# emilemathieu/RiemannHamiltonianMonteCarlo

Hardware: AMD Instinct MI355X
Metric: leapfrog-steps/sec (whole node) (higher is better)
Workload: dtype f64 (the two O(M D^2) contractions as exact int8-sliced integer GEMMs)

## Files before the change

### riemannhamiltonianmontecarlo_amd/csrc/kernels.hip.h

```cpp
#pragma once
#include <hip/hip_runtime.h>
#include <stdint.h>
#include "plan.h"

typedef double d4 __attribute__((ext_vector_type(4)));

#define RM_PI2 6.283185307179586476925286766559
#define RM_PK_DOUBLES (2688 + 64)
template <bool PK>
__device__ __forceinline__ int rm_row(int i) {
  if (!PK) return i * RM_LD;
  const int I = i >> 4;
  return (128 * I + 160) * I + (i & 15) * (16 * I + 18);
}
template <bool PK>
__device__ __forceinline__ int rm_len(int i) { return PK ? 16 * ((i >> 4) + 1) : 64; }

struct DevData {
  const double* Xr;
  const double* Xt;
  const double* t;
  int M, Mp, D, DP, nblk;
  double inv_alpha;
  double log_prior_const;
// ... 584 lines not shown
  }
  double* __restrict__ G = Gq + (size_t)blockIdx.y * plane_stride + (size_t)c * DP * DP;
  int t = 0;
#pragma unroll
  for (int I = 0; I < NB; ++I)
#pragma unroll
    for (int J = I; J < NB; ++J) {
#pragma unroll
      for (int r = 0; r < 4; ++r) {
        const int row = NB * (rr + 4 * r) + I;
        const int col = NB * ci + J;
        double val = acc[t][r];
        if (row == col && blockIdx.y == 0) val += dd.inv_alpha;
        if (I != J || row >= col) {
          G[row * DP + col] = val;
          G[col * DP + row] = val;
        }
      }
      ++t;
    }
}

typedef float f4 __attribute__((ext_vector_type(4)));
template <int NB>
__global__ __launch_bounds__(256) void k_assemble_f32(DevData dd, int n_chains, const int* __restrict__ phase,
                                                      const double* __restrict__ vrow, double* __restrict__ Gq, int nbk) {
  const int DP = dd.DP;
  const int lane = threadIdx.x & 63;
  const int c = blockIdx.x * 4 + (threadIdx.x >> 6);
  if (c >= n_chains) return;
  if (phase[c] != 1) return;
  int bA = 0, bB = 0;
  if (nbk > 1) {
    while ((bB + 1) * (bB + 2) / 2 <= (int)blockIdx.y) ++bB;
    bA = blockIdx.y - bB * (bB + 1) / 2;
  }
  const bool diag = (bA == bB);
  const int WB = 16 * NB;
  const int rr = lane >> 4, ci = lane & 15;
  const double* __restrict__ xpA = dd.Xr + (size_t)rr * DP + WB * bA + NB * ci;
  const double* __restrict__ xpB = dd.Xr + (size_t)rr * DP + WB * bB + NB * ci;
  const double* __restrict__ vp = vrow + (size_t)c * dd.Mp + rr;
  f4 acc[NB][NB];
#pragma unroll
  for (int I = 0; I < NB; ++I)
#pragma unroll
    for (int J = 0; J < NB; ++J) acc[I][J] = (f4){0.f, 0.f, 0.f, 0.f};
  for (int n1 = 0; n1 < dd.Mp; n1 += 16)
#pragma unroll
  for (int n0 = n1; n0 < n1 + 16; n0 += 4) {
    float xa[NB], xb[NB];
    const float vv = (float)vp[n0];
#pragma unroll
    for (int I = 0; I < NB; ++I) {
      xa[I] = vv * (float)xpA[(size_t)n0 * DP + I];
      xb[I] = (float)xpB[(size_t)n0 * DP + I];
    }
#pragma unroll
    for (int I = 0; I < NB; ++I)
#pragma unroll
      for (int J = 0; J < NB; ++J)
        if (!diag || J >= I) acc[I][J] = __builtin_amdgcn_mfma_f32_16x16x4f32(xa[I], xb[J], acc[I][J], 0, 0, 0);
  }
  double* __restrict__ G = Gq + (size_t)c * DP * DP;
#pragma unroll
  for (int I = 0; I < NB; ++I)
#pragma unroll
    for (int J = 0; J < NB; ++J) {
      if (diag && J < I) continue;
#pragma unroll
      for (int r = 0; r < 4; ++r) {
        const int row = WB * bA + NB * (4 * rr + r) + I;
        const int col = WB * bB + NB * ci + J;
        double val = (double)acc[I][J][r];
        if (row == col) val += dd.inv_alpha;
        if (!diag || I != J || row >= col) {
          G[(size_t)row * DP + col] = val;
          G[(size_t)col * DP + row] = val;
        }
      }
    }
}

template <int NB, int CM, bool TRV = false>
__device__ __forceinline__ void mompass_body(const DevData& dd, int n_chains, int nsplit, const double* __restrict__ wq,
                                             const double* __restrict__ uq, double* __restrict__ qpart, d4* __restrict__ ctile,
                                             const double* __restrict__ R = nullptr, double* __restrict__ trpart = nullptr) {
  static_assert(!TRV || CM == 2, "the trace product rides on the pass that loads its c tiles");
  constexpr int DP = 16 * NB;
  constexpr int KK = DP / 4;
  const int lane = threadIdx.x & 63;
  const int c0 = (blockIdx.x * 4 + __builtin_amdgcn_readfirstlane((int)(threadIdx.x >> 6))) * 16;
  if (c0 >= n_chains) return;
  const int split = blockIdx.y;
  const int rr = lane >> 4, ci = lane & 15;
  const int cj = min(c0 + ci, n_chains - 1);
  double Wb[CM == 2 ? 1 : KK], Ub[KK];
#pragma unroll
  for (int kk = 0; kk < KK; ++kk) {
    if (CM != 2) Wb[kk] = wq[(size_t)cj * DP + 4 * kk + rr];
    Ub[kk] = uq[(size_t)cj * DP + 4 * kk + rr];
  }
  __shared__ double s_u[TRV ? 4 * KK * 64 : 1];
  double* const my_u = s_u + (TRV ? ((threadIdx.x >> 6) * KK) * 64 + lane : 0);
  if constexpr (TRV) {
#pragma unroll
    for (int kk = 0; kk < KK; ++kk) my_u[kk * 64] = Ub[kk];
  }
  const brsrc rXt = buf_rsrc(dd.Xt), rXr = buf_rsrc(dd.Xr), rR = buf_rsrc(TRV ? R + (size_t)c0 * dd.Mp : nullptr);
  const unsigned r_off = (unsigned)((cj - c0) * dd.Mp + 8 * rr) * 8u;
  d4 T[TRV ? NB : 1];
  if constexpr (TRV) {
#pragma unroll
    for (int I = 0; I < NB; ++I) T[I] = (d4){0.0, 0.0, 0.0, 0.0};
  }
  const int nb16 = dd.Mp / 16, nb32 = dd.Mp / 32;
  const int per = (nb32 + nsplit - 1) / nsplit;
  const int B0 = split * per, B1 = min(nb32, B0 + per);
  d4* __restrict__ ct = ctile + (size_t)(c0 >> 4) * nb16 * 64 + lane;
  const brsrc rC = buf_rsrc(ctile + (size_t)(c0 >> 4) * nb16 * 64);
  const unsigned c_off = (unsigned)lane * 32u;
  auto load_c = [&](int t) { return buf_d4(rC, c_off, (unsigned)t * 2048u); };
  d4 Q[NB];
#pragma unroll
  for (int I = 0; I < NB; ++I) Q[I] = (d4){0.0, 0.0, 0.0, 0.0};
  const unsigned xt_off = (unsigned)(rr * dd.Mp + 2 * rm_perm16(ci)) * 8u;
  const unsigned xr_off = (unsigned)(8 * rr * DP + NB * ci) * 8u;
  d2 A[KK];
  d4 ccA = (d4){0.0, 0.0, 0.0, 0.0}, ccB = ccA;
  auto load_a = [&](int B, int k0, int k1) {
#pragma unroll
    for (int kk = 0; kk < KK; ++kk)
      if (kk >= k0 && kk < k1) A[kk] = buf_d2(rXt, xt_off, (unsigned)(4 * kk * dd.Mp + B * 32) * 8u);
  };
  auto xrow4 = [&](int n, double (&x)[NB]) { buf_dn<NB>(rXr, xr_off, (unsigned)(n * DP) * 8u, x); };
  if constexpr (CM == 2) {
    double xa[4][NB], xb[4][NB];
    d4 h0 = (d4){0.0, 0.0, 0.0, 0.0}, h1 = h0;
    if (B0 < B1) {
      load_a(B0, 0, KK);
      ccA = load_c(2 * B0);
      ccB = load_c(2 * B0 + 1);
#pragma unroll
      for (int r = 0; r < 4; ++r) xrow4(32 * B0 + 2 * r, xa[r]);
#pragma unroll
      for (int r = 0; r < 4; ++r) xrow4(32 * B0 + 2 * r + 1, xb[r]);
    }
    for (int B = B0; B < B1; ++B) {
      const int Bn = B + 1 < B1 ? B + 1 : B, n1 = 32 * Bn;
      d4 SA = (d4){0.0, 0.0, 0.0, 0.0}, SB = SA;
      if constexpr (TRV) { h0 = buf_d4(rR, r_off, (unsigned)(32 * B) * 8u); h1 = buf_d4(rR, r_off + 32u, (unsigned)(32 * B) * 8u); }
#pragma unroll
      for (int kk = 0; kk < KK; ++kk) {
        const double uk = TRV ? my_u[kk * 64] : Ub[kk];
        SA = __builtin_amdgcn_mfma_f64_16x16x4f64(A[kk].x, uk, SA, 0, 0, 0);
        SB = __builtin_amdgcn_mfma_f64_16x16x4f64(A[kk].y, uk, SB, 0, 0, 0);
        A[kk] = buf_d2(rXt, xt_off, (unsigned)(4 * kk * dd.Mp + Bn * 32) * 8u);
        __builtin_amdgcn_sched_barrier(0);
      }
      double RA[4], RB[4], TA[TRV ? 4 : 1], TB[TRV ? 4 : 1];
#pragma unroll
      for (int r = 0; r < 4; ++r) {
        RA[r] = ccA[r] * SA[r] * SA[r];
        RB[r] = ccB[r] * SB[r] * SB[r];
        if constexpr (TRV) {
          TA[r] = ccA[r] * (r < 2 ? h0[2 * r] : h1[2 * r - 4]);
          TB[r] = ccB[r] * (r < 2 ? h0[2 * r + 1] : h1[2 * r - 3]);
        }
      }
      __builtin_amdgcn_sched_barrier(0);
      ccA = load_c(2 * Bn);
      ccB = load_c(2 * Bn + 1);
      __builtin_amdgcn_sched_barrier(0);
#pragma unroll
      for (int r = 0; r < 4; ++r) {
#pragma unroll
        for (int I = 0; I < NB; ++I) Q[I] = __builtin_amdgcn_mfma_f64_16x16x4f64(xa[r][I], RA[r], Q[I], 0, 0, 0);
        if constexpr (TRV) {
#pragma unroll
          for (int I = 0; I < NB; ++I) T[I] = __builtin_amdgcn_mfma_f64_16x16x4f64(xa[r][I], TA[r], T[I], 0, 0, 0);
        }
        xrow4(n1 + 2 * r, xa[r]);
        __builtin_amdgcn_sched_barrier(0);
      }
#pragma unroll
      for (int r = 0; r < 4; ++r) {
#pragma unroll
        for (int I = 0; I < NB; ++I) Q[I] = __builtin_amdgcn_mfma_f64_16x16x4f64(xb[r][I], RB[r], Q[I], 0, 0, 0);
        if constexpr (TRV) {
#pragma unroll
          for (int I = 0; I < NB; ++I) T[I] = __builtin_amdgcn_mfma_f64_16x16x4f64(xb[r][I], TB[r], T[I], 0, 0, 0);
        }
        xrow4(n1 + 2 * r + 1, xb[r]);
        __builtin_amdgcn_sched_barrier(0);
      }
    }
  } else {
  if (B0 < B1) {
    load_a(B0, 0, KK);
  }
  for (int B = B0; B < B1; ++B) {
    const int n0 = 32 * B;
    double xa[4][NB], xb[4][NB];
    if (CM == 2) {
#pragma unroll
      for (int r = 0; r < 4; ++r) xrow4(n0 + 2 * r, xa[r]);
      __builtin_amdgcn_sched_barrier(0);
    }
    d4 FA = (d4){0.0, 0.0, 0.0, 0.0}, FB = FA, SA = FA, SB = FA;
#pragma unroll
    for (int kk = 0; kk < KK; ++kk) {
      if (CM != 2) {
        FA = __builtin_amdgcn_mfma_f64_16x16x4f64(A[kk].x, Wb[kk], FA, 0, 0, 0);
        FB = __builtin_amdgcn_mfma_f64_16x16x4f64(A[kk].y, Wb[kk], FB, 0, 0, 0);
      }
      const double uk = TRV ? my_u[kk * 64] : Ub[kk];
      SA = __builtin_amdgcn_mfma_f64_16x16x4f64(A[kk].x, uk, SA, 0, 0, 0);
      SB = __builtin_amdgcn_mfma_f64_16x16x4f64(A[kk].y, uk, SB, 0, 0, 0);
    }
    d4 cA = ccA, cB = ccB;
    d4 h0 = (d4){0.0, 0.0, 0.0, 0.0}, h1 = h0;
    if constexpr (TRV) { h0 = buf_d4(rR, r_off, (unsigned)n0 * 8u); h1 = buf_d4(rR, r_off + 32u, (unsigned)n0 * 8u); }
    __builtin_amdgcn_sched_barrier(0);
#pragma unroll
    for (int r = 0; r < 4; ++r) {
      if (CM == 2) xrow4(n0 + 2 * r + 1, xb[r]);
      else xrow4(n0 + 2 * r, xa[r]);
    }
    if (B + 1 < B1) load_a(B + 1, 0, KK / 2);
    __builtin_amdgcn_sched_barrier(0);
    if (CM != 2) {
      d4 pa, va;
      sigmoid4(FA, pa, va, cA);
      if (CM == 1) ct[(size_t)(2 * B) * 64] = cA;
    }
#pragma unroll
    for (int r = 0; r < 4; ++r) {
      const double RA = cA[r] * SA[r] * SA[r];
#pragma unroll
      for (int I = 0; I < NB; ++I) Q[I] = __builtin_amdgcn_mfma_f64_16x16x4f64(xa[r][I], RA, Q[I], 0, 0, 0);
      if constexpr (TRV) {
        const double TA = cA[r] * (r < 2 ? h0[2 * r] : h1[2 * r - 4]);
#pragma unroll
        for (int I = 0; I < NB; ++I) T[I] = __builtin_amdgcn_mfma_f64_16x16x4f64(xa[r][I], TA, T[I], 0, 0, 0);
      }
    }
    __builtin_amdgcn_sched_barrier(0);
    if (CM != 2) {
#pragma unroll
      for (int r = 0; r < 4; ++r) xrow4(n0 + 2 * r + 1, xb[r]);
    }
    if (B + 1 < B1) {
      load_a(B + 1, KK / 2, KK);
      if (CM == 2) { ccA = load_c(2 * B + 2); ccB = load_c(2 * B + 3); }
    }
    __builtin_amdgcn_sched_barrier(0);
    if (CM != 2) {
      d4 pb, vb;
      sigmoid4(FB, pb, vb, cB);
      if (CM == 1) ct[(size_t)(2 * B + 1) * 64] = cB;
    }
#pragma unroll
    for (int r = 0; r < 4; ++r) {
      const double RB = cB[r] * SB[r] * SB[r];
#pragma unroll
      for (int I = 0; I < NB; ++I) Q[I] = __builtin_amdgcn_mfma_f64_16x16x4f64(xb[r][I], RB, Q[I], 0, 0, 0);
      if constexpr (TRV) {
        const double TB = cB[r] * (r < 2 ? h0[2 * r + 1] : h1[2 * r - 3]);
#pragma unroll
        for (int I = 0; I < NB; ++I) T[I] = __builtin_amdgcn_mfma_f64_16x16x4f64(xb[r][I], TB, T[I], 0, 0, 0);
      }
    }
  }
  }
  if (c0 + ci < n_chains) {
    double* __restrict__ out = qpart + ((size_t)split * n_chains + c0 + ci) * DP;
#pragma unroll
    for (int I = 0; I < NB; ++I)
#pragma unroll
      for (int r = 0; r < 4; ++r) {
        const int d = NB * (rr + 4 * r) + I;
        if (d < dd.D) out[d] = Q[I][r];
      }
    if constexpr (TRV) {
      double* __restrict__ tout = trpart + ((size_t)split * n_chains + c0 + ci) * DP;
#pragma unroll
      for (int I = 0; I < NB; ++I)
#pragma unroll
        for (int r = 0; r < 4; ++r) {
          const int d = NB * (rr + 4 * r) + I;
          if (d < dd.D) tout[d] = T[I][r];
        }
    }
  }
}
template <int NB>
__global__ __launch_bounds__(256, 2) void k_mompass_trv(DevData dd, int n_chains, int nsplit, const double* __restrict__ uq, double* __restrict__ qpart,
                                                     d4* __restrict__ ctile, const double* __restrict__ R, double* __restrict__ trpart) {
  mompass_body<NB, 2, true>(dd, n_chains, nsplit, nullptr, uq, qpart, ctile, R, trpart);
}
template <int NB, int CM>
__global__ __launch_bounds__(256, 2) void k_mompass(DevData dd, int n_chains, int nsplit, const double* __restrict__ wq,
                                                 const double* __restrict__ uq, double* __restrict__ qpart, d4* __restrict__ ctile,
                                                 const int* __restrict__ cstale = nullptr) {
  if constexpr (CM == 3) {
    const int c0 = (blockIdx.x * 4 + (threadIdx.x >> 6)) * 16;
    if (c0 >= n_chains) return;
    const int c = c0 + (threadIdx.x & 15);
    const bool stale = __builtin_amdgcn_ballot_w64(c < n_chains && cstale[min(c, n_chains - 1)] != 0) != 0ull;
    if (stale) mompass_body<NB, 1>(dd, n_chains, nsplit, wq, uq, qpart, ctile);
    else mompass_body<NB, 2>(dd, n_chains, nsplit, wq, uq, qpart, ctile);
  } else {
    mompass_body<NB, CM>(dd, n_chains, nsplit, wq, uq, qpart, ctile);
  }
}

template <int NB>
__global__ __launch_bounds__(256, 2) void k_crestore(DevData dd, int n_chains, const int* __restrict__ phase,
                                                  const double* __restrict__ wq, d4* __restrict__ ctile, int* __restrict__ cstale,
                                                  const int* __restrict__ list, const int* __restrict__ count) {
  constexpr int DP = 16 * NB;
  constexpr int KK = DP / 4;
  const int lane = threadIdx.x & 63;
  const int cnt = min(*count, n_chains);
  const int split = blockIdx.y, nsplit = gridDim.y;
  const int rr = lane >> 4, ci = lane & 15;
  for (int g16 = (blockIdx.x * 4 + (threadIdx.x >> 6)) * 16; g16 < cnt; g16 += gridDim.x * 64) {
  const int chn = list[min(g16 + ci, cnt - 1)];
  const int cj = min(max(chn, 0), n_chains - 1);
  const bool live = g16 + ci < cnt && chn >= 0 && chn < n_chains && phase[cj] == 1;
  double Wb[KK];
#pragma unroll
  for (int kk = 0; kk < KK; ++kk) Wb[kk] = wq[(size_t)cj * DP + 4 * kk + rr];
  const int nb16 = dd.Mp / 16, nb32 = dd.Mp / 32;
  const int per = (nb32 + nsplit - 1) / nsplit;
  const int B0 = split * per, B1 = min(nb32, B0 + per);
  const double* __restrict__ xt_p = dd.Xt + (size_t)rr * dd.Mp + 2 * rm_perm16(ci);
  d4* __restrict__ ct = ctile + (size_t)(cj >> 4) * nb16 * 64 + rr * 16 + (cj & 15);
  d2 A[KK];
  auto load_a = [&](int B) {
#pragma unroll
    for (int kk = 0; kk < KK; ++kk) A[kk] = *(const d2*)(xt_p + (size_t)(4 * kk) * dd.Mp + B * 32);
  };
  if (B0 < B1) load_a(B0);
  for (int B = B0; B < B1; ++B) {
    d4 FA = (d4){0.0, 0.0, 0.0, 0.0}, FB = FA;
    __builtin_amdgcn_sched_barrier(0);
#pragma unroll
    for (int kk = 0; kk < KK; ++kk) {
      FA = __builtin_amdgcn_mfma_f64_16x16x4f64(A[kk].x, Wb[kk], FA, 0, 0, 0);
      FB = __builtin_amdgcn_mfma_f64_16x16x4f64(A[kk].y, Wb[kk], FB, 0, 0, 0);
    }
    __builtin_amdgcn_sched_barrier(0);
    if (B + 1 < B1) load_a(B + 1);
    __builtin_amdgcn_sched_barrier(0);
    d4 cA, cB, pa, va, pb, vb;
    sigmoid4(FA, pa, va, cA);
    sigmoid4(FB, pb, vb, cB);
    if (live) {
      ct[(size_t)(2 * B) * 64] = cA;
      ct[(size_t)(2 * B + 1) * 64] = cB;
    }
  }
  if (live && rr == 0 && split == 0) cstale[cj] = 0;
  }
}

template <int NB>
__global__ __launch_bounds__(256) void k_leverage(DevData dd, int n_chains, const int* __restrict__ phase,
                                                  const double* __restrict__ Ginv, const double* __restrict__ crow,
                                                  double* __restrict__ tr, double* __restrict__ trpart) {
  constexpr int DP = 16 * NB;
  const int lane = threadIdx.x & 63;
  const int c = blockIdx.x * 4 + (threadIdx.x >> 6);
  if (c >= n_chains) return;
  if (phase[c] != 1) return;
  const int rr = lane >> 4, ci = lane & 15;
  const double* __restrict__ Gi = Ginv + (size_t)c * DP * DP;
  double Gv[NB][4][NB];
#pragma unroll
  for (int I = 0; I < NB; ++I)
#pragma unroll
    for (int s = 0; s < 4; ++s)
#pragma unroll
      for (int J = 0; J < NB; ++J) {
        const int row = NB * (4 * s + rr) + I, col = NB * ci + J;
        Gv[I][s][J] = (J >= I) ? Gi[row * DP + col] * (I == J ? 1.0 : 2.0) : 0.0;
      }
  const double* __restrict__ xp = dd.Xr + (size_t)ci * DP + NB * rr;
  const double* __restrict__ cp = crow + (size_t)c * dd.Mp + ci;
  double tracc[4][NB];
#pragma unroll
  for (int r = 0; r < 4; ++r)
#pragma unroll
    for (int J = 0; J < NB; ++J) tracc[r][J] = 0.0;

// ... 1087 lines not shown
```

### riemannhamiltonianmontecarlo_amd/csrc/plan.h

```cpp
#pragma once
#include "../../include/rmhmc.h"

#include <stddef.h>
#include <stdint.h>
#include <string.h>

#include <algorithm>

#define RM_LD 66

#define FS_D 8
#define FS_WAVES 4
#define FS_PT 104

#define MS_MAXMP 2048
#define MS_GLD 34

template <int NB>
constexpr int ms_lds_doubles(int Mp) {
  return 64 * RM_LD + 32 * MS_GLD + 4 * (16 * NB) * (16 * NB) + 2 * Mp + 12 * 32 + 4 * 40;
}

#define I8_BM 128
constexpr int i8_tile_wn(int S) { return S <= 6 ? 4 : 2; }
constexpr int i8_tile_tn(int) { return 1; }

#define AMH_MAX_ONCHIP_ROWS (256 * 48)

struct Options {
  int64_t graph = 1, sorted = 1, inflight = 32, cdyn = 1, crestore = 1, i8_force_rebase = 0;
  int64_t ccache = 1, medium = 1, fused = 1, hmc_traj_maxn = -1, fsplit = 0, nsplit_max = 64, nsplit_waves = -1, i8_tail = -1,
          i8_delta = 1, i8_delta_inner = 1, i8_zdirect = 3;
};
struct OptionDesc { const char* key; int64_t Options::*slot; bool create_only; int64_t lo, hi; };
inline const OptionDesc kOptions[] = {
    {"graph", &Options::graph, false, 0, 1},
    {"sorted", &Options::sorted, false, 0, 1},
    {"inflight", &Options::inflight, false, 0, 1 << 20},
    {"cdyn", &Options::cdyn, false, 0, 1},
    {"crestore", &Options::crestore, false, 0, 1},
    {"i8_force_rebase", &Options::i8_force_rebase, false, 0, 1},
    {"ccache", &Options::ccache, true, 0, 1},
    {"medium", &Options::medium, true, 0, 1},
    {"fused", &Options::fused, true, 0, 1},
    {"hmc_traj_maxn", &Options::hmc_traj_maxn, true, -1, (int64_t)1 << 40},
    {"fsplit", &Options::fsplit, true, 0, 64},
    {"nsplit_max", &Options::nsplit_max, true, 1, 1 << 20},
    {"nsplit_waves", &Options::nsplit_waves, true, -1, 1 << 20},
    {"i8_tail", &Options::i8_tail, true, -1, 1},
    {"i8_delta", &Options::i8_delta, true, 0, 1},
    {"i8_delta_inner", &Options::i8_delta_inner, true, 0, 1},
    {"i8_zdirect", &Options::i8_zdirect, true, 0, 3},
};
inline const OptionDesc* find_option(const char* key) {
  if (!key) return nullptr;
  for (const OptionDesc& d : kOptions)
    if (!strcmp(d.key, key)) return &d;
  return nullptr;
}
enum OptionError { OPT_OK, OPT_UNKNOWN, OPT_CREATE_ONLY, OPT_RANGE };
inline OptionError check_option(const OptionDesc* d, int64_t value, bool at_create) {
  if (!d) return OPT_UNKNOWN;
  if (d->create_only && !at_create) return OPT_CREATE_ONLY;
  if (value < d->lo || value > d->hi) return OPT_RANGE;
  return OPT_OK;
}

struct PlanCheck { int code; const char* msg; };
inline PlanCheck plan_check(int64_t M, int32_t D, int64_t n_chains, int32_t dtype, uint32_t flags) {
  auto no = [](int code, const char* m) { return PlanCheck{code, m}; };
  if (M <= 0 || D <= 0 || n_chains <= 0) return no(RMHMC_ERR_INVALID, "rmhmc_create: bad shape");
  if (dtype != RMHMC_F64) return no(RMHMC_ERR_UNSUPPORTED, "rmhmc_create: only float64 is built (the reference is float64)");
  if (D > 256) return no(RMHMC_ERR_UNSUPPORTED, "rmhmc_create: D > 256 is not supported (64 < D <= 256 uses the blocked large-D path)");
  if (flags & RMHMC_FLAG_ORACLE_LITERAL) return no(RMHMC_ERR_UNSUPPORTED, "rmhmc_create: the literal variant exists only in the CPU oracle");
  if (M > (int64_t)1 << 30 || n_chains > (int64_t)1 << 30) return no(RMHMC_ERR_UNSUPPORTED, "rmhmc_create: M or n_chains too large");
  if (D <= 64 && (M + 63) / 64 * 64 * (int64_t)(16 * ((D + 15) / 16)) * 8 >= (int64_t)1 << 32)
    return no(RMHMC_ERR_UNSUPPORTED, "rmhmc_create: the data matrix of the D <= 64 path must stay below 4 GB");
  return no(RMHMC_OK, "");
}

struct Plan {
  int64_t M = 0, n = 0;
  int D = 0, DP = 0, NB = 0, Mp = 0, nblk = 0;
  bool big = false;
  int nbk = 1, npairs = 1;
  int nsplit = 1;
  int fsplit = 1;
  int gpart_planes = 0;
  bool hpart_at_create = false;
  bool i8_requested = false;
  int i8S = 0, i8_nks = 0, i8_bn = 128, i8_chunk = 1;
  int NP = 0, NPp = 0;
  int i8_nkp = 0, i8_NRp = 0;
  int nCp = 0;
  int ksplit_a = 1, ksplit_l = 1;
  bool tail_acc = false;
  bool tail_always = false;
  int tail_pieces = 1, tail_blocks = 0;
  bool gbase = false;
  bool i8_lev_full = false;
  bool fused = false;
  size_t fused_lds = 0;
  bool medium = false;
  size_t medium_lds = 0;
  bool hmc_traj = false;
};

inline Plan make_plan(int64_t M, int32_t D, int64_t n_chains, uint32_t flags, const Options& opt) {
  Plan p;
  p.M = M; p.D = D; p.n = n_chains;
  p.NB = (D + 15) / 16; p.DP = 16 * p.NB;
  if (D > 64) {
    p.big = true;
    p.nbk = (D + 63) / 64;
    p.npairs = p.nbk * (p.nbk + 1) / 2;
    p.DP = 64 * p.nbk;
    p.NB = 4;
  }
  p.Mp = (int)((M + 63) / 64 * 64); p.nblk = p.Mp / 64;
  {
    const long long cgroups = (n_chains + 15) / 16, nb16 = p.Mp / 16;
    const long long target = opt.nsplit_waves > 0 ? opt.nsplit_waves : (p.big ? 6144 : 2048);
    long long ns = (target + cgroups - 1) / cgroups;
    if (ns < 1) ns = 1;
    if (ns > nb16) ns = nb16;
    if (ns > opt.nsplit_max) ns = opt.nsplit_max;
    p.nsplit = (int)ns;
    if (!p.big) {
      const long long waves = n_chains;
      long long fs = waves >= 1024 ? 1 : std::min<long long>(16, (2048 + waves - 1) / waves);
      fs = std::min<long long>(fs, std::max(1, p.Mp / 256));
      if (opt.fsplit >= 1) fs = opt.fsplit;
      p.fsplit = (int)fs;
    }
  }
// ... 80 lines not shown
```

### riemannhamiltonianmontecarlo_amd/csrc/rmhmc_hip.hip

```cpp
#include "../../include/rmhmc.h"
#include "../../include/rmhmc_amh.h"
#include "../../include/rmhmc_iwls.h"
#include "../../include/rmhmc_gibbs.h"
#include "../../include/rmhmc_out.h"
#include "../../include/rmhmc_diag.h"
#include "../../include/rmhmc_phmc.h"
#include "../../include/rmhmc_adapt.h"
#include "../../include/rmhmc_ais.h"
#include "../../include/rmhmc_pred.h"
#include "../../include/rmhmc_smc.h"
#include "../../include/rmhmc_quant.h"
#include "plan.h"
#include "mass.h"
#include "kernels.hip.h"
#include "fused_small.hip.h"
#include "large_d.hip.h"
#include "metric_i8.hip.h"
#include "medium_step.hip.h"
#include "amh.hip.h"
#include "iwls.hip.h"
#include "gibbs.hip.h"
#include "output.hip.h"
#include "diag.hip.h"
#include "phmc.hip.h"
// ... 340 lines not shown
    else
      hipLaunchKernelGGL((k_leverage_i8<S, WN, TN>), grid, dim3(128 * WN), (i8_lds_bytes<S, WN, TN>()), st, args...);
  };
  if (ctx->ksplit_l > 1) {
    const size_t plane = (size_t)g.n * ctx->Mp;
    tiles(dim3(nblk, (unsigned)ctx->ksplit_l), (const int8_t*)g.Qs, (const int8_t*)ctx->d_Zt, g.nCp, ctx->i8_NRp, ctx->i8_nkp, 0, ctx->i8_nkp, 0,
          (ctx->big || g.ctile) ? 0 : 1, g.n, ctx->Mp, (const int*)g.ch.phase, (const double*)g.qscale, (const double*)ctx->d_zscale,
          (const double*)g.ch.rv2, g.Rpart, plane);
    hipLaunchKernelGGL(k_sum_planes, dim3((unsigned)((plane + 255) / 256)), dim3(256), 0, st, g.ch.rv0, g.Rpart, ctx->ksplit_l, plane, plane);
    return;
  }
  for (int kp0 = 0; kp0 < ctx->i8_nkp; kp0 += ctx->i8_chunk) {
    const int nk = std::min(ctx->i8_chunk, ctx->i8_nkp - kp0);
    tiles(dim3(nblk), (const int8_t*)g.Qs, (const int8_t*)ctx->d_Zt, g.nCp, ctx->i8_NRp, ctx->i8_nkp, kp0, nk, kp0 > 0 ? 1 : 0,
          (ctx->big || g.ctile) ? 0 : 1, g.n, ctx->Mp, (const int*)g.ch.phase, (const double*)g.qscale, (const double*)ctx->d_zscale,
          (const double*)g.ch.rv2, g.ch.rv0, (size_t)0);
  }
}
void launch_assemble(rmhmc_ctx* ctx, Group& g, const double* v, bool inner = false, bool delta = false, bool keep_base = false) {
  if (ctx->i8 && delta && ctx->big)
    launch(ctx, "vsplit", [&](hipStream_t st) { launch_assemble_i8_t<6, 4, 1>(ctx, g, v, st, 0, true); });
  if (ctx->i8 && delta && inner) {
    launch(ctx, "assemble_i8_inner_delta", [&](hipStream_t st) { launch_assemble_i8_delta(ctx, g, st, 5); });
    return;
  }
  if (ctx->i8 && delta) {
    launch(ctx, "assemble_i8_delta", [&](hipStream_t st) { launch_assemble_i8_delta(ctx, g, st, 6); });
    return;
  }
  if (ctx->i8) {
    if (ctx->big)
      launch(ctx, "vsplit", [&](hipStream_t st) { I8_SWITCH(ctx, (launch_assemble_i8_t<S_, WN_, TN_>(ctx, g, v, st, 0))); });
    const int suse = (inner && ctx->i8_inner_drop && ctx->i8S == 6) ? 5 : ctx->i8S;
    launch(ctx, suse == ctx->i8S ? "assemble_i8" : "assemble_i8_inner", [&](hipStream_t st) {
      I8_SWITCH_S(suse, (launch_assemble_i8_t<S_, WN_, TN_>(ctx, g, v, st, 1)));
      if (keep_base && ctx->big && g.Gbase)
        (void)hipMemcpyAsync(g.Gbase, g.ch.Gq, sizeof(double) * (size_t)g.n * ctx->DP * ctx->DP, hipMemcpyDeviceToDevice, st);
    });
    return;
  }
  launch(ctx, "assemble", [&](hipStream_t st) {
    if (ctx->flags & RMHMC_FLAG_FP32_METRIC) {
      if (ctx->big) {
        hipLaunchKernelGGL((k_assemble_f32<4>), dim3((unsigned)((g.n + 3) / 4), ctx->npairs), dim3(256), 0, st, ctx->dd, g.n, g.ch.phase, v,
                           g.ch.Gq, ctx->nbk);
      } else {
        NB_SWITCH(ctx, hipLaunchKernelGGL((k_assemble_f32<NB_>), dim3((unsigned)((g.n + 3) / 4)), dim3(256), 0, st, ctx->dd, g.n,
                                          g.ch.phase, v, g.ch.Gq, 1));
      }
      return;
    }
    if (ctx->big) {
      hipLaunchKernelGGL(k_assemble_pair<false>, dim3((unsigned)((g.n + 3) / 4), ctx->npairs - ctx->nbk), dim3(256), 0, st, ctx->dd, g.n,
                         g.ch.phase, v, g.ch.Gq);
      hipLaunchKernelGGL(k_assemble_pair<true>, dim3((unsigned)((g.n + 3) / 4), ctx->nbk), dim3(256), 0, st, ctx->dd, g.n, g.ch.phase, v,
                         g.ch.Gq);
      return;
    }
    if (ctx->fsplit > 1) {
      const size_t plane = (size_t)g.n * ctx->DP * ctx->DP;
      dim3 grid((unsigned)((g.n + 3) / 4), (unsigned)ctx->fsplit);
      NB_SWITCH(ctx, hipLaunchKernelGGL((k_assemble<NB_>), grid, dim3(256), 0, st, ctx->dd, g.n, g.ch.phase, v, g.Gpart, plane));
      hipLaunchKernelGGL(k_sum_planes, dim3((unsigned)((plane + 255) / 256)), dim3(256), 0, st, g.ch.Gq, g.Gpart, ctx->fsplit, plane, plane);
      return;
    }
    dim3 grid((unsigned)((g.n + 3) / 4));
    NB_SWITCH(ctx, hipLaunchKernelGGL((k_assemble<NB_>), grid, dim3(256), 0, st, ctx->dd, g.n, g.ch.phase, v, g.ch.Gq, (size_t)0));
  });
}

void launch_mompass(rmhmc_ctx* ctx, Group& g, const double* w, int cmode) {
  launch(ctx, "mompass", [&](hipStream_t st) {
    if (!ctx->opt.ccache) cmode = 0;
    if (ctx->big) {
      dim3 grid((unsigned)((g.n + 15) / 16), ctx->nsplit);
      switch (cmode) {
        case 1: hipLaunchKernelGGL(k_mompass_big<1>, grid, dim3(256), 0, st, ctx->dd, g.n, ctx->nsplit, ctx->nbk, w, g.ch.uq, g.ch.qpart, g.ctile); break;
        case 2: hipLaunchKernelGGL(k_mompass_big<2>, grid, dim3(256), 0, st, ctx->dd, g.n, ctx->nsplit, ctx->nbk, w, g.ch.uq, g.ch.qpart, g.ctile); break;
        default: hipLaunchKernelGGL(k_mompass_big<0>, grid, dim3(256), 0, st, ctx->dd, g.n, ctx->nsplit, ctx->nbk, w, g.ch.uq, g.ch.qpart, g.ctile); break;
      }
      return;
    }
    dim3 grid((unsigned)((g.n + 63) / 64), ctx->nsplit);
    switch (cmode) {
      case 1:
        if (ctx->opt.cdyn) { NB_SWITCH(ctx, hipLaunchKernelGGL((k_mompass<NB_, 3>), grid, dim3(256), 0, st, ctx->dd, g.n, ctx->nsplit, w, g.ch.uq, g.ch.qpart, g.ctile, g.ch.cstale)); }
        else { NB_SWITCH(ctx, hipLaunchKernelGGL((k_mompass<NB_, 1>), grid, dim3(256), 0, st, ctx->dd, g.n, ctx->nsplit, w, g.ch.uq, g.ch.qpart, g.ctile)); }
        break;
      case 2: NB_SWITCH(ctx, hipLaunchKernelGGL((k_mompass<NB_, 2>), grid, dim3(256), 0, st, ctx->dd, g.n, ctx->nsplit, w, g.ch.uq, g.ch.qpart, g.ctile)); break;
      default: NB_SWITCH(ctx, hipLaunchKernelGGL((k_mompass<NB_, 0>), grid, dim3(256), 0, st, ctx->dd, g.n, ctx->nsplit, w, g.ch.uq, g.ch.qpart, g.ctile)); break;
    }
  });
}

static bool fused_trace(const rmhmc_ctx* ctx, const Group& g) { return ctx->i8 && !ctx->big && g.ctile != nullptr && ctx->opt.ccache; }

void launch_leverage(rmhmc_ctx* ctx, Group& g, int part = 0) {
  if (ctx->i8 && part == 2) {
    launch(ctx, "small", [&](hipStream_t st) {
      hipLaunchKernelGGL(k_reduce_tr, dim3((unsigned)g.n), dim3(64), 0, st, ctx->D, ctx->DP, g.ch, g.ch.gpart, ctx->nsplit);
    });
    return;
  }
  if (ctx->i8) {
    launch(ctx, "qsplit", [&](hipStream_t st) { I8_SWITCH(ctx, (launch_leverage_i8_t<S_, WN_, TN_>(ctx, g, st, 0))); });
    const int suse = (ctx->i8_inner_drop && ctx->i8S == 6 && !ctx->i8_lev_full) ? 5 : ctx->i8S;
    launch(ctx, "leverage_i8", [&](hipStream_t st) { I8_SWITCH_S(suse, (launch_leverage_i8_t<S_, WN_, TN_>(ctx, g, st, 1))); });
    if (part == 1) return;
    launch(ctx, "trvec", [&](hipStream_t st) {
      if (ctx->big) {
        dim3 grid((unsigned)((g.n + 15) / 16), ctx->nsplit);
        hipLaunchKernelGGL(k_trace_big, grid, dim3(256), 0, st, ctx->dd, g.n, ctx->nsplit, ctx->nbk, 1, g.ch.rv2, g.ch.rv0, g.ch.gpart);
        return;
      }
      dim3 grid((unsigned)((g.n + 63) / 64), ctx->nsplit);
      NB_SWITCH(ctx, hipLaunchKernelGGL((k_trvec<NB_>), grid, dim3(256), 0, st, ctx->dd, g.n, ctx->nsplit, g.ch.rv0, g.ch.gpart, (const d4*)g.ctile));
    });
    launch(ctx, "small", [&](hipStream_t st) {
      hipLaunchKernelGGL(k_reduce_tr, dim3((unsigned)g.n), dim3(64), 0, st, ctx->D, ctx->DP, g.ch, g.ch.gpart, ctx->nsplit);
    });
    return;
  }
  if (ctx->big) {
    double* hpart = ctx->d_hpart;
    launch(ctx, "leverage", [&](hipStream_t st) {
      hipLaunchKernelGGL(k_leverage_pair<false>, dim3((unsigned)((g.n + 3) / 4), ctx->npairs - ctx->nbk), dim3(256), 0, st, ctx->dd, g.n,
                         ctx->nbk, g.ch.phase, g.ch.trj.Ginv, hpart);
      hipLaunchKernelGGL(k_leverage_pair<true>, dim3((unsigned)((g.n + 3) / 4), ctx->nbk), dim3(256), 0, st, ctx->dd, g.n, ctx->nbk,
                         g.ch.phase, g.ch.trj.Ginv, hpart);
    });
    launch(ctx, "leverage", [&](hipStream_t st) {
      dim3 grid((unsigned)((g.n + 15) / 16), ctx->nsplit);
      hipLaunchKernelGGL(k_trace_big, grid, dim3(256), 0, st, ctx->dd, g.n, ctx->nsplit, ctx->nbk, ctx->npairs, g.ch.rv2, hpart, g.ch.gpart);
    });
    launch(ctx, "small", [&](hipStream_t st) {
      hipLaunchKernelGGL(k_reduce_tr, dim3((unsigned)g.n), dim3(64), 0, st, ctx->D, ctx->DP, g.ch, g.ch.gpart, ctx->nsplit);
    });
    return;
  }
  const int fs = std::min(ctx->fsplit, ctx->nsplit);
  launch(ctx, "leverage", [&](hipStream_t st) {
    dim3 grid((unsigned)((g.n + 3) / 4), (unsigned)fs);
    NB_SWITCH(ctx, hipLaunchKernelGGL((k_leverage<NB_>), grid, dim3(256), 0, st, ctx->dd, g.n, g.ch.phase, g.ch.trj.Ginv, g.ch.rv2,
                                      g.ch.trj.tr, g.ch.gpart));
  });
  if (fs > 1)
    launch(ctx, "small", [&](hipStream_t st) {
      hipLaunchKernelGGL(k_reduce_tr, dim3((unsigned)g.n), dim3(64), 0, st, ctx->D, ctx->DP, g.ch, g.ch.gpart, fs);
    });
}

#define SMALL(ctx, g, name, kern, ...)                                                                     \
  launch(ctx, name, [&](hipStream_t st_) { hipLaunchKernelGGL(kern, dim3((unsigned)(g).n), dim3(64), 0, st_, __VA_ARGS__); })

#define BIG(ctx, g, name, kern, ...)                                                                       \
  launch(ctx, name, [&](hipStream_t st_) { hipLaunchKernelGGL(kern, dim3((unsigned)(g).n), dim3(256), 0, st_, __VA_ARGS__); })

void eval_point_phases(rmhmc_ctx* ctx, Group& g, const Run* step, int mode = 0, bool want_G = false) {
  const double eps = step ? step->eps : 0.0;
  const bool delta = step && use_delta(ctx, *step, g);
  launch_rowpass<RP_F>(ctx, g, g.ch.trj.w, g.ch.rv0, g.ch.rv2, delta);
  if (ctx->big) SMALL(ctx, g, "small", k_finish_big, ctx->dd, g.ch, ctx->nsplit);
  launch_assemble(ctx, g, g.ch.rv0, false, delta);
  if (ctx->big) {
    if (want_G)
      (void)hipMemcpyAsync(ctx->d_Gcopy, g.ch.Gq, sizeof(double) * (size_t)g.n * ctx->DP * ctx->DP, hipMemcpyDeviceToDevice, ctx->stream);
    BIG(ctx, g, "factor", k_chol_big<1>, ctx->dd, g.ch, ctx->nbk, ctx->d_Wd, eps);
    BIG(ctx, g, "factor", k_inverse_big, ctx->dd, g.ch, ctx->nbk, ctx->d_Wd);
    SMALL(ctx, g, "small", k_ginv_matvec, ctx->D, ctx->DP, g.ch, g.ch.p);
  } else {
    launch(ctx, "factor", [&](hipStream_t st) {
      NB_SWITCH(ctx, hipLaunchKernelGGL((k_factor_full<NB_>), dim3((unsigned)g.n), dim3(64), 0, st, ctx->dd, g.ch, ctx->nsplit));
    });
  }
  if (mode == 1) return;
  if (mode == 2) {
    launch_leverage(ctx, g);
    return;
  }
  if (fused_trace(ctx, g)) {
    launch_leverage(ctx, g, 1);
    launch(ctx, "mompass", [&](hipStream_t st) {
      dim3 grid((unsigned)((g.n + 63) / 64), ctx->nsplit);
      NB_SWITCH(ctx, hipLaunchKernelGGL((k_mompass_trv<NB_>), grid, dim3(256), 0, st, ctx->dd, g.n, ctx->nsplit, g.ch.uq, g.ch.qpart, g.ctile, g.ch.rv0, g.ch.gpart));
    });
  } else {
    launch_mompass(ctx, g, g.ch.trj.w, 2);
    launch_leverage(ctx, g);
  }
  SMALL(ctx, g, "small", k_mom_final, ctx->D, ctx->DP, g.ch, eps, step ? 1 : 0, ctx->nsplit, fused_trace(ctx, g) ? g.ch.gpart : (const double*)nullptr);
}

template <int NB>
void launch_step_medium_nb(rmhmc_ctx* ctx, Group& g, hipStream_t st, int guards, const Run* step, int fold, const IterParams& ip) {
  const double eps = step ? step->eps : 0.0;
  const int K = step ? step->K : 0, eval_only = step ? 0 : 1;
  const int rpt = (ctx->Mp + 255) / 256;
  const dim3 grid((unsigned)g.n), block(256);
  const size_t lds = ctx->medium_lds;
  switch (rpt * 16 * NB <= 64 ? rpt : 0) {
    case 1: hipLaunchKernelGGL((k_step_medium<NB, 1>), grid, block, lds, st, ctx->dd, g.ch, eps, K, guards, eval_only, fold, ip); break;
    case 2: hipLaunchKernelGGL((k_step_medium<NB, 2>), grid, block, lds, st, ctx->dd, g.ch, eps, K, guards, eval_only, fold, ip); break;
    case 3: hipLaunchKernelGGL((k_step_medium<NB, (NB == 1 ? 3 : 0)>), grid, block, lds, st, ctx->dd, g.ch, eps, K, guards, eval_only, fold, ip); break;
    case 4: hipLaunchKernelGGL((k_step_medium<NB, (NB == 1 ? 4 : 0)>), grid, block, lds, st, ctx->dd, g.ch, eps, K, guards, eval_only, fold, ip); break;
    default: hipLaunchKernelGGL((k_step_medium<NB, 0>), grid, block, lds, st, ctx->dd, g.ch, eps, K, guards, eval_only, fold, ip); break;
  }
}
void launch_step_medium(rmhmc_ctx* ctx, Group& g, hipStream_t st, int guards, const Run* step, int fold, const IterParams& ip) {
  if (ctx->NB == 1) launch_step_medium_nb<1>(ctx, g, st, guards, step, fold, ip);
  else launch_step_medium_nb<2>(ctx, g, st, guards, step, fold, ip);
}

void step_phases(rmhmc_ctx* ctx, const Run& run, Group& g) {
  const int D = ctx->D, DP = ctx->DP, K = run.K;
  const double eps = run.eps;
  const int guards = (ctx->flags & RMHMC_FLAG_GUARDS) ? 1 : 0;
  if (ctx->medium) {
    launch(ctx, "medium", [&](hipStream_t st) { launch_step_medium(ctx, g, st, guards, &run, 0, IterParams{}); });
    return;
  }
  if (!ctx->big && ctx->opt.cdyn && g.ctile && g.ch.stale_list)
    launch(ctx, "mompass", [&](hipStream_t st) {
      const int rsplit = std::max(1, std::min(32, ctx->Mp / 32 / 4));
      dim3 grid((unsigned)std::min((g.n + 63) / 64, 8), (unsigned)rsplit);
      NB_SWITCH(ctx, hipLaunchKernelGGL((k_crestore<NB_>), grid, dim3(256), 0, st, ctx->dd, g.n, g.ch.phase, g.ch.trj.w, g.ctile, g.ch.cstale,
                                        g.ch.stale_list, g.ch.stale_count));
    });
  const bool fuse = !ctx->big;
  for (int it = 0; it < K; ++it) {
    if (it == 0 || !fuse) SMALL(ctx, g, "small", k_ginv_matvec, D, DP, g.ch, it == 0 ? g.ch.p : g.ch.PM);
    launch_mompass(ctx, g, g.ch.trj.w, it == 0 ? 1 : 2);
    if (!fuse) SMALL(ctx, g, "small", k_mom_update, D, DP, g.ch, eps, it == K - 1 ? 1 : 0, ctx->nsplit);
    else if (it < K - 1) SMALL(ctx, g, "small", k_mom_update_matvec, D, DP, g.ch, eps, ctx->nsplit);
  }
  if (ctx->big) {
    SMALL(ctx, g, "small", k_ginv_matvec, D, DP, g.ch, g.ch.p);
    SMALL(ctx, g, "small", k_pos_first_big, D, DP, g.ch, eps);
  } else {
    SMALL(ctx, g, "factor", k_pos_first, D, DP, g.ch, eps, ctx->nsplit);
  }
  for (int it = 1; it < K; ++it) {
    launch_rowpass<RP_V>(ctx, g, g.ch.wq, g.ch.rv0, nullptr, use_delta_inner(ctx, run, g, it));
    const bool base = (it == 1 && use_delta_inner(ctx, run, g, 2)) || (it == K - 1 && use_delta(ctx, run, g));
    launch_assemble(ctx, g, g.ch.rv0, it < K - 1, use_delta_inner(ctx, run, g, it), base);
    if (ctx->big)
      BIG(ctx, g, "factor", k_chol_big<0>, ctx->dd, g.ch, ctx->nbk, ctx->d_Wd, eps);
    else
      launch(ctx, "factor", [&](hipStream_t st) {
        NB_SWITCH(ctx, hipLaunchKernelGGL((k_factor_solve<NB_>), dim3((unsigned)g.n), dim3(64), 0, st, D, DP, g.ch, eps, it == K - 1 ? guards : -1));
      });
  }
  if (ctx->big || K < 2) SMALL(ctx, g, "small", k_pos_final, D, DP, g.ch, guards);
  eval_point_phases(ctx, g, &run);
}

IterParams iter_params(rmhmc_ctx* ctx, const Run& run, const IterBase& b) {
  IterParams ip{};
  ip.flags = ctx->flags;
  ip.L = run.L;
  ip.seed = run.seed;
  ip.chain_offset = run.chain_offset;
  ip.iter_limit = b.limit;
  ip.burn_in = b.burn_in;
  ip.S = b.S;
  ip.samples = b.samples;
  ip.orig = run.orig;
  if (b.explicit_rng) {
// ... 2614 lines not shown
```

Baseline: 579,700.

## Reuse transposed Xt tile via per-wave LDS instead of refetching Xr rows

In the CM 2 momentum pass, the Xt fragments already loaded for the S products are written into a per-wave swizzled LDS tile, then read back as the Xr row operands for the Q and T accumulations. This removes the separate global fetch of Xr rows. With XP on, the u operand in the trace variant stays in registers instead of LDS. The cost is extra LDS space, wave-level fences, and LDS traffic, which may affect occupancy under launch bounds of 2. The path is enabled by default through a new xpose option.

```diff
diff --git a/riemannhamiltonianmontecarlo_amd/csrc/kernels.hip.h b/riemannhamiltonianmontecarlo_amd/csrc/kernels.hip.h
--- a/riemannhamiltonianmontecarlo_amd/csrc/kernels.hip.h
+++ b/riemannhamiltonianmontecarlo_amd/csrc/kernels.hip.h
@@ -690,11 +690,33 @@
     }
 }
 
-template <int NB, int CM, bool TRV = false>
+template <int NB>
+struct XTile {
+  static constexpr int DP = 16 * NB;
+  static constexpr int RS = NB == 4 ? DP : DP + 2;
+  static constexpr int SIZE = 32 * RS;
+  __device__ static __forceinline__ int pos(int row, int col) {
+    if constexpr (NB == 4) {
+      const int p = row >> 1, g = (p & 3) | ((p >> 3) << 2);
+      return row * RS + ((col & 2) << 4) + (((col >> 2) ^ g) << 1) + (col & 1);
+    } else {
+      return row * RS + col;
+    }
+  }
+};
+__device__ __forceinline__ void xtile_sync() {
+  __builtin_amdgcn_fence(__ATOMIC_RELEASE, "wavefront");
+  __builtin_amdgcn_wave_barrier();
+  __builtin_amdgcn_fence(__ATOMIC_ACQUIRE, "wavefront");
+}
+template <int NB, int CM, bool TRV = false, bool XP = false>
 __device__ __forceinline__ void mompass_body(const DevData& dd, int n_chains, int nsplit, const double* __restrict__ wq,
                                              const double* __restrict__ uq, double* __restrict__ qpart, d4* __restrict__ ctile,
                                              const double* __restrict__ R = nullptr, double* __restrict__ trpart = nullptr) {
   static_assert(!TRV || CM == 2, "the trace product rides on the pass that loads its c tiles");
+  static_assert(!XP || CM == 2, "the transposed fetch is built into the CM 2 loop");
+  constexpr bool ULDS = TRV && !XP;
+  constexpr int XP_AHEAD = TRV ? 1 : 2;
   constexpr int DP = 16 * NB;
   constexpr int KK = DP / 4;
   const int lane = threadIdx.x & 63;
@@ -709,9 +731,9 @@
     if (CM != 2) Wb[kk] = wq[(size_t)cj * DP + 4 * kk + rr];
     Ub[kk] = uq[(size_t)cj * DP + 4 * kk + rr];
   }
-  __shared__ double s_u[TRV ? 4 * KK * 64 : 1];
-  double* const my_u = s_u + (TRV ? ((threadIdx.x >> 6) * KK) * 64 + lane : 0);
-  if constexpr (TRV) {
+  __shared__ double s_u[ULDS ? 4 * KK * 64 : 1];
+  double* const my_u = s_u + (ULDS ? ((threadIdx.x >> 6) * KK) * 64 + lane : 0);
+  if constexpr (ULDS) {
 #pragma unroll
     for (int kk = 0; kk < KK; ++kk) my_u[kk * 64] = Ub[kk];
   }
@@ -742,6 +764,23 @@
       if (kk >= k0 && kk < k1) A[kk] = buf_d2(rXt, xt_off, (unsigned)(4 * kk * dd.Mp + B * 32) * 8u);
   };
   auto xrow4 = [&](int n, double (&x)[NB]) { buf_dn<NB>(rXr, xr_off, (unsigned)(n * DP) * 8u, x); };
+  typedef XTile<NB> XT;
+  __shared__ __attribute__((aligned(16))) double s_x[XP ? 4 * XT::SIZE : 1];
+  double* const my_x = s_x + (XP ? (threadIdx.x >> 6) * XT::SIZE : 0);
+  auto tput = [&](int kk) {
+    my_x[XT::pos(2 * rm_perm16(ci), 4 * kk + rr)] = A[kk].x;
+    my_x[XT::pos(2 * rm_perm16(ci) + 1, 4 * kk + rr)] = A[kk].y;
+  };
+  auto tget = [&](int i, double (&x)[NB]) {
+    const int row = 8 * rr + 2 * (i & 3) + (i >> 2);
+    if constexpr (NB == 4) {
+      const d2 lo = *(const d2*)(my_x + XT::pos(row, 4 * ci)), hi = *(const d2*)(my_x + XT::pos(row, 4 * ci + 2));
+      x[0] = lo.x; x[1] = lo.y; x[2] = hi.x; x[3] = hi.y;
+    } else {
+#pragma unroll
+      for (int I = 0; I < NB; ++I) x[I] = my_x[XT::pos(row, NB * ci + I)];
+    }
+  };
   if constexpr (CM == 2) {
     double xa[4][NB], xb[4][NB];
     d4 h0 = (d4){0.0, 0.0, 0.0, 0.0}, h1 = h0;
@@ -749,10 +788,12 @@
       load_a(B0, 0, KK);
       ccA = load_c(2 * B0);
       ccB = load_c(2 * B0 + 1);
-#pragma unroll
-      for (int r = 0; r < 4; ++r) xrow4(32 * B0 + 2 * r, xa[r]);
-#pragma unroll
-      for (int r = 0; r < 4; ++r) xrow4(32 * B0 + 2 * r + 1, xb[r]);
+      if constexpr (!XP) {
+#pragma unroll
+        for (int r = 0; r < 4; ++r) xrow4(32 * B0 + 2 * r, xa[r]);
+#pragma unroll
+        for (int r = 0; r < 4; ++r) xrow4(32 * B0 + 2 * r + 1, xb[r]);
+      }
     }
     for (int B = B0; B < B1; ++B) {
       const int Bn = B + 1 < B1 ? B + 1 : B, n1 = 32 * Bn;
@@ -760,10 +801,20 @@
       if constexpr (TRV) { h0 = buf_d4(rR, r_off, (unsigned)(32 * B) * 8u); h1 = buf_d4(rR, r_off + 32u, (unsigned)(32 * B) * 8u); }
 #pragma unroll
       for (int kk = 0; kk < KK; ++kk) {
-        const double uk = TRV ? my_u[kk * 64] : Ub[kk];
+        const double uk = ULDS ? my_u[kk * 64] : Ub[kk];
         SA = __builtin_amdgcn_mfma_f64_16x16x4f64(A[kk].x, uk, SA, 0, 0, 0);
         SB = __builtin_amdgcn_mfma_f64_16x16x4f64(A[kk].y, uk, SB, 0, 0, 0);
+        if constexpr (XP) {
+          asm volatile("" : "+v"(SA), "+v"(SB));
+          tput(kk);
+        }
         A[kk] = buf_d2(rXt, xt_off, (unsigned)(4 * kk * dd.Mp + Bn * 32) * 8u);
+        __builtin_amdgcn_sched_barrier(0);
+      }
+      if constexpr (XP) {
+        xtile_sync();
+#pragma unroll
+        for (int i = 0; i < XP_AHEAD; ++i) tget(i, xa[i]);
         __builtin_amdgcn_sched_barrier(0);
       }
       double RA[4], RB[4], TA[TRV ? 4 : 1], TB[TRV ? 4 : 1];
@@ -788,7 +839,9 @@
 #pragma unroll
           for (int I = 0; I < NB; ++I) T[I] = __builtin_amdgcn_mfma_f64_16x16x4f64(xa[r][I], TA[r], T[I], 0, 0, 0);
         }
-        xrow4(n1 + 2 * r, xa[r]);
+        if constexpr (!XP) xrow4(n1 + 2 * r, xa[r]);
+        else if (r + XP_AHEAD < 4) tget(r + XP_AHEAD, xa[r + XP_AHEAD]);
+        else tget(r + XP_AHEAD, xb[r + XP_AHEAD - 4]);
         __builtin_amdgcn_sched_barrier(0);
       }
 #pragma unroll
@@ -799,9 +852,11 @@
 #pragma unroll
           for (int I = 0; I < NB; ++I) T[I] = __builtin_amdgcn_mfma_f64_16x16x4f64(xb[r][I], TB[r], T[I], 0, 0, 0);
         }
-        xrow4(n1 + 2 * r + 1, xb[r]);
+        if constexpr (!XP) xrow4(n1 + 2 * r + 1, xb[r]);
+        else if (r + XP_AHEAD < 4) tget(4 + r + XP_AHEAD, xb[r + XP_AHEAD]);
         __builtin_amdgcn_sched_barrier(0);
       }
+      if constexpr (XP) xtile_sync();
     }
   } else {
   if (B0 < B1) {
@@ -822,7 +877,7 @@
         FA = __builtin_amdgcn_mfma_f64_16x16x4f64(A[kk].x, Wb[kk], FA, 0, 0, 0);
         FB = __builtin_amdgcn_mfma_f64_16x16x4f64(A[kk].y, Wb[kk], FB, 0, 0, 0);
       }
-      const double uk = TRV ? my_u[kk * 64] : Ub[kk];
+      const double uk = ULDS ? my_u[kk * 64] : Ub[kk];
       SA = __builtin_amdgcn_mfma_f64_16x16x4f64(A[kk].x, uk, SA, 0, 0, 0);
       SB = __builtin_amdgcn_mfma_f64_16x16x4f64(A[kk].y, uk, SB, 0, 0, 0);
     }
@@ -902,12 +957,12 @@
     }
   }
 }
-template <int NB>
+template <int NB, bool XP = false>
 __global__ __launch_bounds__(256, 2) void k_mompass_trv(DevData dd, int n_chains, int nsplit, const double* __restrict__ uq, double* __restrict__ qpart,
                                                      d4* __restrict__ ctile, const double* __restrict__ R, double* __restrict__ trpart) {
-  mompass_body<NB, 2, true>(dd, n_chains, nsplit, nullptr, uq, qpart, ctile, R, trpart);
-}
-template <int NB, int CM>
+  mompass_body<NB, 2, true, XP>(dd, n_chains, nsplit, nullptr, uq, qpart, ctile, R, trpart);
+}
+template <int NB, int CM, bool XP = false>
 __global__ __launch_bounds__(256, 2) void k_mompass(DevData dd, int n_chains, int nsplit, const double* __restrict__ wq,
                                                  const double* __restrict__ uq, double* __restrict__ qpart, d4* __restrict__ ctile,
                                                  const int* __restrict__ cstale = nullptr) {
@@ -917,9 +972,9 @@
     const int c = c0 + (threadIdx.x & 15);
     const bool stale = __builtin_amdgcn_ballot_w64(c < n_chains && cstale[min(c, n_chains - 1)] != 0) != 0ull;
     if (stale) mompass_body<NB, 1>(dd, n_chains, nsplit, wq, uq, qpart, ctile);
-    else mompass_body<NB, 2>(dd, n_chains, nsplit, wq, uq, qpart, ctile);
+    else mompass_body<NB, 2, false, XP>(dd, n_chains, nsplit, wq, uq, qpart, ctile);
   } else {
-    mompass_body<NB, CM>(dd, n_chains, nsplit, wq, uq, qpart, ctile);
+    mompass_body<NB, CM, false, XP>(dd, n_chains, nsplit, wq, uq, qpart, ctile);
   }
 }
 
diff --git a/riemannhamiltonianmontecarlo_amd/csrc/plan.h b/riemannhamiltonianmontecarlo_amd/csrc/plan.h
--- a/riemannhamiltonianmontecarlo_amd/csrc/plan.h
+++ b/riemannhamiltonianmontecarlo_amd/csrc/plan.h
@@ -30,7 +30,7 @@
 struct Options {
   int64_t graph = 1, sorted = 1, inflight = 32, cdyn = 1, crestore = 1, i8_force_rebase = 0;
   int64_t ccache = 1, medium = 1, fused = 1, hmc_traj_maxn = -1, fsplit = 0, nsplit_max = 64, nsplit_waves = -1, i8_tail = -1,
-          i8_delta = 1, i8_delta_inner = 1, i8_zdirect = 3;
+          i8_delta = 1, i8_delta_inner = 1, i8_zdirect = 3, xpose = 1;
 };
 struct OptionDesc { const char* key; int64_t Options::*slot; bool create_only; int64_t lo, hi; };
 inline const OptionDesc kOptions[] = {
@@ -51,6 +51,7 @@
     {"i8_delta", &Options::i8_delta, true, 0, 1},
     {"i8_delta_inner", &Options::i8_delta_inner, true, 0, 1},
     {"i8_zdirect", &Options::i8_zdirect, true, 0, 3},
+    {"xpose", &Options::xpose, true, 0, 1},
 };
 inline const OptionDesc* find_option(const char* key) {
   if (!key) return nullptr;
diff --git a/riemannhamiltonianmontecarlo_amd/csrc/rmhmc_hip.hip b/riemannhamiltonianmontecarlo_amd/csrc/rmhmc_hip.hip
--- a/riemannhamiltonianmontecarlo_amd/csrc/rmhmc_hip.hip
+++ b/riemannhamiltonianmontecarlo_amd/csrc/rmhmc_hip.hip
@@ -446,12 +446,17 @@
       return;
     }
     dim3 grid((unsigned)((g.n + 63) / 64), ctx->nsplit);
+    const bool xp = (ctx->opt.xpose & 1) != 0;
     switch (cmode) {
       case 1:
-        if (ctx->opt.cdyn) { NB_SWITCH(ctx, hipLaunchKernelGGL((k_mompass<NB_, 3>), grid, dim3(256), 0, st, ctx->dd, g.n, ctx->nsplit, w, g.ch.uq, g.ch.qpart, g.ctile, g.ch.cstale)); }
+        if (ctx->opt.cdyn && xp) { NB_SWITCH(ctx, hipLaunchKernelGGL((k_mompass<NB_, 3, true>), grid, dim3(256), 0, st, ctx->dd, g.n, ctx->nsplit, w, g.ch.uq, g.ch.qpart, g.ctile, g.ch.cstale)); }
+        else if (ctx->opt.cdyn) { NB_SWITCH(ctx, hipLaunchKernelGGL((k_mompass<NB_, 3>), grid, dim3(256), 0, st, ctx->dd, g.n, ctx->nsplit, w, g.ch.uq, g.ch.qpart, g.ctile, g.ch.cstale)); }
         else { NB_SWITCH(ctx, hipLaunchKernelGGL((k_mompass<NB_, 1>), grid, dim3(256), 0, st, ctx->dd, g.n, ctx->nsplit, w, g.ch.uq, g.ch.qpart, g.ctile)); }
         break;
-      case 2: NB_SWITCH(ctx, hipLaunchKernelGGL((k_mompass<NB_, 2>), grid, dim3(256), 0, st, ctx->dd, g.n, ctx->nsplit, w, g.ch.uq, g.ch.qpart, g.ctile)); break;
+      case 2:
+        if (xp) { NB_SWITCH(ctx, hipLaunchKernelGGL((k_mompass<NB_, 2, true>), grid, dim3(256), 0, st, ctx->dd, g.n, ctx->nsplit, w, g.ch.uq, g.ch.qpart, g.ctile)); }
+        else { NB_SWITCH(ctx, hipLaunchKernelGGL((k_mompass<NB_, 2>), grid, dim3(256), 0, st, ctx->dd, g.n, ctx->nsplit, w, g.ch.uq, g.ch.qpart, g.ctile)); }
+        break;
       default: NB_SWITCH(ctx, hipLaunchKernelGGL((k_mompass<NB_, 0>), grid, dim3(256), 0, st, ctx->dd, g.n, ctx->nsplit, w, g.ch.uq, g.ch.qpart, g.ctile)); break;
     }
   });
@@ -546,7 +551,11 @@
     launch_leverage(ctx, g, 1);
     launch(ctx, "mompass", [&](hipStream_t st) {
       dim3 grid((unsigned)((g.n + 63) / 64), ctx->nsplit);
-      NB_SWITCH(ctx, hipLaunchKernelGGL((k_mompass_trv<NB_>), grid, dim3(256), 0, st, ctx->dd, g.n, ctx->nsplit, g.ch.uq, g.ch.qpart, g.ctile, g.ch.rv0, g.ch.gpart));
+      if (ctx->opt.xpose & 1) {
+        NB_SWITCH(ctx, hipLaunchKernelGGL((k_mompass_trv<NB_, true>), grid, dim3(256), 0, st, ctx->dd, g.n, ctx->nsplit, g.ch.uq, g.ch.qpart, g.ctile, g.ch.rv0, g.ch.gpart));
+      } else {
+        NB_SWITCH(ctx, hipLaunchKernelGGL((k_mompass_trv<NB_>), grid, dim3(256), 0, st, ctx->dd, g.n, ctx->nsplit, g.ch.uq, g.ch.qpart, g.ctile, g.ch.rv0, g.ch.gpart));
+      }
     });
   } else {
     launch_mompass(ctx, g, g.ch.trj.w, 2);
```

New measurement: 583,400 (median of 3 runs). No clear change (+0.6%).
